# llrtt/G-NeRF

Measured on NVIDIA B200. Metric: ray-samples/sec, higher is better.
Workload: dtype f32

## Files before the change

### g-nerf_b200/csrc/tpr_render_ws.cuh

```cuda
#pragma once
#include <cuda_runtime.h>
#include <stdint.h>
#include <stddef.h>
#include <string.h>
#include <cuda_bf16.h>
#include "triplane_b200.h"
#include "tpr_render.cuh"
#include "tpr_ws.cuh"

namespace tpr {
using namespace tc;

namespace ws {

struct Barriers {
  uint64_t a1_full[kBufs];
  uint64_t a1_free[kBufs];
  uint64_t d1_full;
  uint64_t a2_full;
  uint64_t coarse_ready[kCtx];
  uint64_t fine_ready[kCtx];
  uint64_t csig_ready[kCtx];
  uint64_t fsig_ready[kCtx];
  uint64_t stg_full[2];
};

struct Ctx { float* dep; float* sig; float* u; float* ray; int* rk; };

struct Geom { long long ray0; int n, rstride, nr; };
__device__ __forceinline__ Geom group_geom(const RenderArgs& a, unsigned grp, int R) {
  Geom g;
  const unsigned tpi = (unsigned)a.tiles_per_img;
  const unsigned n = grp / tpi, gi = grp - n * tpi;
  const bool colm = a.col_w > 0;
  const unsigned cw = colm ? (unsigned)a.col_w : 1u;
  const unsigned gy = gi / cw, gx = gi - gy * cw;
  g.n = (int)n;
  g.ray0 = (long long)n * a.rays_per_img + (colm ? (long long)(gy * R * cw + gx) : (long long)gi * R);
  g.rstride = (int)cw;
  g.nr = colm ? R : (int)min((long long)R, a.rays_per_img - (long long)gi * R);
  return g;
}

template <int MODE, bool TRAIN = false>
__device__ __forceinline__ void gather_tile(const RenderArgs& a, float* a1_hi, const float* __restrict__ img,
                                            const Ctx& cx, Tap2* tw, int nr, int Dx, int off, int S, int t, int dpt_shift,
                                            int warp, int lane, long long ray0 = 0, int rstride = 0) {
#ifndef TPR_GATHER_256
  const int grp = lane >> 3, sub = lane & 7;
#endif
  const int dpt = 1 << dpt_shift;
  {
    const int s = lane / 3, p = lane - s * 3;
    const int row = warp * 8 + s;
    const int r = row >> dpt_shift, di = t * dpt + (row & (dpt - 1));
    if (lane < 24 && r < nr && di < Dx) {
      const float d = cx.dep[r * S + off + di];
      const float* ry = cx.ray + r * 8;
      const float px = __fmul_rn(__fadd_rn(ry[0], __fmul_rn(d, ry[3])), a.box_scale);
      const float py = __fmul_rn(__fadd_rn(ry[1], __fmul_rn(d, ry[4])), a.box_scale);
      const float pz = __fmul_rn(__fadd_rn(ry[2], __fmul_rn(d, ry[5])), a.box_scale);
      Taps tp;
      plane_taps(p == 2 ? pz : px, p == 0 ? py : (p == 1 ? pz : px), a.H, a.W, tp);
      const int po = p * a.H * a.W * kC;
      *reinterpret_cast<uint4*>(tw[lane].off) = make_uint4((unsigned)(tp.off[0] + po) >> 2, (unsigned)(tp.off[1] + po) >> 2,
                                                           (unsigned)(tp.off[2] + po) >> 2, (unsigned)(tp.off[3] + po) >> 2);
      *reinterpret_cast<float4*>(tw[lane].w2) = make_float4(tp.w[0], tp.w[0], tp.w[1], tp.w[1]);
      *reinterpret_cast<float4*>(tw[lane].w2 + 4) = make_float4(tp.w[2], tp.w[2], tp.w[3], tp.w[3]);
    }
  }
  __syncwarp();
#ifdef TPR_GATHER_256
  {
    const int s = lane >> 2, sub4 = lane & 3;
    const ulonglong2* base = reinterpret_cast<const ulonglong2*>(img) + 2 * sub4;
    asm volatile("" : "+l"(base));
    const int row = warp * 8 + s;
    const int r = row >> dpt_shift, di = t * dpt + (row & (dpt - 1));
    if (r < nr && di < Dx) {
      float4* keep = (TRAIN && a.sample_features != nullptr)
          ? reinterpret_cast<float4*>(a.sample_features + ((ray0 + (long long)r * rstride) * S + off + di) * 32) + 2 * sub4 : nullptr;
      blend_sample8<MODE>(a1_hi, base, tw + s * 3, row, sub4, keep);
    }
  }
#else
  const ulonglong2* base = reinterpret_cast<const ulonglong2*>(img) + sub;
  asm volatile("" : "+l"(base));
#pragma unroll 1
  for (int rd = 0; rd < 2; ++rd) {
#if !defined(TPR_ROWS_INTERLEAVED) || TPR_ROWS_INTERLEAVED
    const int s = (grp & 1) | ((grp >> 1) << 2) | (rd << 1);
#else
    const int s = rd * 4 + grp;
#endif
    const int row = warp * 8 + s;
    const int r = row >> dpt_shift, di = t * dpt + (row & (dpt - 1));
    if (r < nr && di < Dx) {
      const Tap2* te = tw + s * 3;
      float4* keep = (TRAIN && a.sample_features != nullptr)
          ? reinterpret_cast<float4*>(a.sample_features + ((ray0 + (long long)r * rstride) * S + off + di) * 32) + sub : nullptr;
      blend_sample<MODE>(a1_hi, base, te, row, sub, keep);
    }
  }
#endif
  __syncwarp();
}

template <int MODE, int E, int ER, bool PROF, bool TRAIN = false>
__global__ void __launch_bounds__(kThreads, 1) render_ws_kernel(const RenderArgs a) {
  extern __shared__ uint8_t smem_raw[];
  uint8_t* base = smem_raw + ((1024u - (smem_u32(smem_raw) & 1023u)) & 1023u);
  Tiles<MODE>& tl = *reinterpret_cast<Tiles<MODE>*>(base);
  Tap2* taps = reinterpret_cast<Tap2*>(base + sizeof(Tiles<MODE>));
  float* fl = reinterpret_cast<float*>(base + sizeof(Tiles<MODE>) + sizeof(Tap2) * kGatherWarps * 24);
  const int R = a.R, Dc = a.Dc, Df = a.Df, S = Dc + Df;
  const int dpt_shift = R == 8 ? 4 : 5, dpt = 1 << dpt_shift;
  const int ctx_floats = 2 * R * S + R * Df + R * 8 + (R == 4 ? R * Df : 0);
  float* scratch = fl + kCtx * ctx_floats;
  auto ctx_of = [&](int gi) {
    float* p = fl + (gi & (kCtx - 1)) * ctx_floats;
    Ctx c; c.dep = p; c.sig = p + R * S; c.u = c.sig + R * S; c.ray = c.u + R * Df; c.rk = reinterpret_cast<int*>(c.ray + R * 8);
    return c;
  };
  __shared__ Barriers bars;
  __shared__ uint32_t tmem_base_sm;
  __shared__ unsigned range_sm[2];
  __shared__ unsigned freed_warps;
  __shared__ int slot_tab[kCtx][16];
  __shared__ long long prof[24];
  const bool profiling = PROF && a.dbg != nullptr && blockIdx.x == 0;
#define PROF_T0() long long pt0_ = (PROF && profiling) ? clock64() : 0
#define PROF_ADD(i, cond) do { if (PROF && profiling && (cond)) { const long long now_ = clock64(); prof[i] += now_ - pt0_; pt0_ = now_; } } while (0)
  const int tid = threadIdx.x, warp = __shfl_sync(0xffffffffu, tid >> 5, 0), lane = tid & 31;
  const bool sleep_waits = (a.variant & 2) != 0;
#define WAIT_SLACK(bar, par) do { if (sleep_waits) mbar_wait_sleep(bar, par); else mbar_wait_parked(bar, par); } while (0)

  const int nf_host = a.Df;
  if (tid == 0) {
    range_sm[0] = 0xffffffffu; range_sm[1] = 0u;
    for (int b = 0; b < kBufs; ++b) { mbar_init(&bars.a1_full[b], kGatherWarps); mbar_init(&bars.a1_free[b], 1); }
    mbar_init(&bars.d1_full, 1); mbar_init(&bars.a2_full, kDecodeWarps);
    mbar_init(&bars.stg_full[0], 1); mbar_init(&bars.stg_full[1], 1);
    for (int c = 0; c < kCtx; ++c) {
      mbar_init(&bars.coarse_ready[c], kRayWarps); mbar_init(&bars.fine_ready[c], kRayWarps);
      mbar_init(&bars.csig_ready[c], nf_host == 0 ? 5 : 4); mbar_init(&bars.fsig_ready[c], 5);
    }
    freed_warps = 0u;
    for (int i = 0; i < 24; ++i) prof[i] = 0;
    fence_mbar_init();
  }
  if (warp == 0) { tmem_alloc(&tmem_base_sm, 512); tmem_relinquish(); }
  for (int i = tid; i < (int)(sizeof(tl.a1) / 16); i += kThreads) reinterpret_cast<float4*>(tl.a1)[i] = make_float4(0.f, 0.f, 0.f, 0.f);
  stage_weights<MODE>(a.dec, tl);
  fence_proxy_async_smem();
  tcgen05_fence_before();
  __syncthreads();
  tcgen05_fence_after();
  const uint32_t tmem = __shfl_sync(0xffffffffu, tmem_base_sm, 0);
  const uint32_t lane_base = (uint32_t)((warp & 3) * 32) << 16;

  const int nc = (Dc + dpt - 1) >> dpt_shift, nf = Df > 0 ? (Df + dpt - 1) >> dpt_shift : 0;
  const int G = (int)((a.n_tiles - blockIdx.x + gridDim.x - 1) / gridDim.x);
  const size_t img_stride = (size_t)3 * a.H * a.W * kC;
  const bool per_ray = a.rs != nullptr;

  if (warp < kGatherWarps) {
    Tap2* tw = taps + warp * 24;
    int b = 0; uint32_t ph = 0;
    for (int step = 0; step <= G; ++step) {
#pragma unroll 1
      for (int jb = 0; jb < 2; ++jb) {
        const int pass = jb;
        int gi;
        if (pass == 0) { if (step >= G) continue; gi = step; }
        else { if (step < 1 || nf == 0) continue; gi = step - 1; }
        const Geom gg = group_geom(a, blockIdx.x + (unsigned)gi * gridDim.x, R);
        const Ctx cx = ctx_of(gi);
        const uint32_t cpar = (uint32_t)(gi >> 2) & 1u;
        PROF_T0();
        WAIT_SLACK(pass == 0 ? &bars.coarse_ready[gi & 3] : &bars.fine_ready[gi & 3], cpar);
        PROF_ADD(pass, tid == 0);
        const float* img = a.planes + (size_t)((unsigned)gg.n % (unsigned)a.plane_sets) * img_stride;
        const int T = pass == 0 ? nc : nf, Dx = pass == 0 ? Dc : Df, off = pass == 0 ? 0 : Dc;
#pragma unroll 1
        for (int t = 0; t < T; ++t) {
          WAIT_SLACK(&bars.a1_free[b], ph ^ 1u);
          PROF_ADD(2, tid == 0);
          gather_tile<MODE, TRAIN>(a, tl.a1[b][0], img, cx, tw, gg.nr, Dx, off, S, t, dpt_shift, warp, lane, gg.ray0, gg.rstride);
          fence_proxy_async_smem();
          __syncwarp();
          if (lane == 0) mbar_arrive(&bars.a1_full[b]);
          PROF_ADD(3, tid == 0);
          if (++b == kBufs) { b = 0; ph ^= 1u; }
        }
      }
    }
  } else if (warp < kFirstRayWarp) {
    const int dw = warp - kFirstDecodeWarp, q = dw & 3, h = dw >> 2;
    const bool issuer = dw == 0;
    uint32_t pt = 0;
    const uint32_t dbase = smem_desc_lo(smem_u32(&tl));
    uint32_t free_mask = (1u << Cols<MODE>::ns) - 1u;
    int freed_groups = 0;
    int b = 0; uint32_t ph = 0;
    for (int step = 0; step <= G; ++step) {
#pragma unroll 1
      for (int jb = 0; jb < 2; ++jb) {
        const int pass = jb;
        int gi;
        if (pass == 0) { if (step >= G) continue; gi = step; }
        else { if (step < 1 || nf == 0) continue; gi = step - 1; }
        const Geom gg = group_geom(a, blockIdx.x + (unsigned)gi * gridDim.x, R);
        const Ctx cx = ctx_of(gi);
        const int T = pass == 0 ? nc : nf, Dx = pass == 0 ? Dc : Df, off = pass == 0 ? 0 : Dc;
#pragma unroll 1
        for (int t = 0; t < T; ++t) {
          PROF_T0();
          const bool pl = dw == 0 && lane == 0;
          const uint32_t st = tmem;
          if (issuer) {
            mbar_wait_parked(&bars.a1_full[b], ph);
            PROF_ADD(4, pl);
            tcgen05_fence_after();
            const int bu = __shfl_sync(0xffffffffu, b, 0);
            if (elect_one_sync()) {
              issue_layer1<MODE>(dbase, bu, st);
              mma_commit(&bars.a1_free[b]);
              mma_commit(&bars.d1_full);
            }
            __syncwarp();
          }
          if (++b == kBufs) { b = 0; ph ^= 1u; }
          int slot = 0;
          if (issuer) {
            do {
              const int fg = (int)(*reinterpret_cast<volatile unsigned*>(&freed_warps) / kRayWarps);
              for (; freed_groups < fg; ++freed_groups)
                for (int i = 0; i < nc + nf; ++i) free_mask |= 1u << slot_tab[freed_groups & (kCtx - 1)][i];
            } while (free_mask == 0u);
            __threadfence_block();
            slot = __shfl_sync(0xffffffffu, __ffs(free_mask) - 1, 0);
            free_mask &= ~(1u << slot);
            if (lane == 0) slot_tab[gi & (kCtx - 1)][(pass == 0 ? 0 : nc) + t] = slot;
          }
          PROF_ADD(5, pl);
          mbar_wait_parked(&bars.d1_full, pt);
          PROF_ADD(6, pl);
          tcgen05_fence_after();
          const float sgp = epilogue1<MODE>(tl, st, lane_base, h);
          tcgen05_fence_before();
          __syncwarp();
          if (lane == 0) mbar_arrive(&bars.a2_full);
          PROF_ADD(7, pl);
          if (issuer) {
            mbar_wait_parked(&bars.a2_full, pt);
            PROF_ADD(8, pl);
            tcgen05_fence_after();
            if (elect_one_sync()) {
              issue_layer2<MODE>(dbase, st, tmem + Cols<MODE>::slots + slot * kSlotCols);
              if (t == T - 1 && (pass == 1 || nf == 0)) mma_commit(pass == 0 ? &bars.csig_ready[gi & 3] : &bars.fsig_ready[gi & 3]);
            }
            __syncwarp();
          }
          PROF_ADD(9, pl);
          float* ps = tl.psig + (pt ? kRows : 0);
          if (h == 1) ps[q * 32 + lane] = sgp;
          named_bar_sync(3 + q, 64);
          if (h == 0) {
            const int row = q * 32 + lane, r = row >> dpt_shift, di = t * dpt + (row & (dpt - 1));
            if (r < gg.nr && di < Dx) cx.sig[r * S + off + di] = sgp + ps[row] + tl.bias2[kNc];
          }
          PROF_ADD(10, pl);
          if (h == 0 && t == T - 1) {
            __syncwarp();
            if (lane == 0) mbar_arrive(pass == 0 ? &bars.csig_ready[gi & 3] : &bars.fsig_ready[gi & 3]);
          }
          pt ^= 1u;
          PROF_ADD(11, pl);
        }
      }
    }
  } else {
    const int rw = warp - kFirstRayWarp, rtid = tid - kFirstRayWarp * 32;
    const int q = rw & 3, hc = rw >> 2;
    constexpr int kRayThreads = kRayWarps * 32;
    float* wa = scratch; float* wb = wa + R * S; float* wc = wb + R * S; float* rayw = wc + R * S;
    float mn = __int_as_float(0x7f800000), mx = -__int_as_float(0x7f800000);
    float smn = mn, smx = mx;
    int cur_slot = 0;
#define RAY_SYNC() named_bar_sync(2, kRayThreads)

    const bool pl = rtid == 0;
    const bool bulk = a.bulk_inputs != 0;
    float* stg_jit = rayw + R; float* stg_u = stg_jit + 2 * R * Dc; float* stg_ray = stg_u + 2 * R * Df;
    int* hist = reinterpret_cast<int*>(stg_ray + R * 8 + 8);
    const bool merge = R == 4 && nf > 0 && (Df & 3) == 0 && a.variant != 3;
    const bool split = merge && a.noise_c == nullptr && (a.variant & 16) == 0;
    float* so_a = split ? reinterpret_cast<float*>(hist + R * (Dc + 4)) : wa;
    float* so_b = split ? so_a + R * S : wb;
    auto prefetch = [&](int gi) {
      const Geom gg = group_geom(a, blockIdx.x + (unsigned)gi * gridDim.x, R);
      if (rtid < gg.nr * 6) {
        const int r = rtid / 6, c = rtid - r * 6;
        const long long g = gg.ray0 + (long long)r * gg.rstride;
        cp_async4(stg_ray + rtid, c < 3 ? a.origins + g * 3 + c : a.dirs + g * 3 + c - 3);
      }
      float* sj = stg_jit + (gi & 1) * R * Dc; float* su = stg_u + (gi & 1) * R * Df;
      if (bulk) {
        if (rtid == 0) {
          mbar_arrive_expect_tx(&bars.stg_full[gi & 1], (uint32_t)(gg.nr * (Dc + Df)) * 4u);
          for (int r = 0; r < gg.nr; ++r) {
            const long long g = gg.ray0 + (long long)r * gg.rstride;
            bulk_copy_g2s(sj + r * Dc, a.jitter + g * Dc, (uint32_t)Dc * 4u, &bars.stg_full[gi & 1]);
            if (Df > 0) bulk_copy_g2s(su + r * Df, a.u + g * Df, (uint32_t)Df * 4u, &bars.stg_full[gi & 1]);
          }
        }
      } else {
        for (int s = rtid; s < gg.nr * Dc; s += kRayThreads) {
          const int r = s / Dc, k = s - r * Dc;
          cp_async4(sj + s, a.jitter + (gg.ray0 + (long long)r * gg.rstride) * Dc + k);
        }
        for (int s = rtid; s < gg.nr * Df; s += kRayThreads) {
          const int r = s / Df, k = s - r * Df;
          cp_async4(su + s, a.u + (gg.ray0 + (long long)r * gg.rstride) * Df + k);
        }
      }
      cp_async_commit();
    };
    auto setup = [&](int gi) {
      PROF_T0();
      const Geom gg = group_geom(a, blockIdx.x + (unsigned)gi * gridDim.x, R);
      const Ctx cx = ctx_of(gi);
      cp_async_wait_all();
      if (bulk) mbar_wait_parked(&bars.stg_full[gi & 1], (uint32_t)(gi >> 1) & 1u);
      const float* sj = stg_jit + (gi & 1) * R * Dc; const float* su = stg_u + (gi & 1) * R * Df;
      if (rtid < gg.nr * 6) { const int r = rtid / 6; cx.ray[r * 8 + (rtid - r * 6)] = stg_ray[rtid]; }
      for (int s = rtid; s < gg.nr * Dc; s += kRayThreads) {
        const int r = s / Dc, k = s - r * Dc;
        const long long g = gg.ray0 + (long long)r * gg.rstride;
        const float lo = per_ray ? __ldg(a.rs + g) : a.ray_start, hi = per_ray ? __ldg(a.re + g) : a.ray_end;
        cx.dep[r * S + k] = coarse_depth(a, k, sj[s], lo, hi, per_ray);
      }
      for (int s = rtid; s < gg.nr * Df; s += kRayThreads) cx.u[s] = su[s];
      __syncwarp();
      if (lane == 0) mbar_arrive(&bars.coarse_ready[gi & 3]);
      PROF_ADD(12, pl);
    };

    auto resample = [&](int gi) {
      const Geom gg = group_geom(a, blockIdx.x + (unsigned)gi * gridDim.x, R);
      const Ctx cx = ctx_of(gi);
      PROF_T0();
      WAIT_SLACK(&bars.csig_ready[gi & 3], (uint32_t)(gi >> 2) & 1u);
      PROF_ADD(13, pl);
      if (a.noise_c != nullptr) {
        add_density_noise(a, a.noise_c, cx.sig, S, 0, Dc, gg.nr * Dc, gg.ray0, gg.rstride, rtid, kRayThreads);
        RAY_SYNC();
      }
      for (int r = rw; r < gg.nr; r += kRayWarps)
        warp_resample_ray(a, cx.dep + r * S, cx.sig + r * S, wa + r * S, wb + r * S, wc + r * S, cx.dep + r * S + Dc,
                          gg.ray0 + (long long)r * gg.rstride, lane, cx.u + r * Df);
      if (!split && merge && rw >= 4 && rw - 4 < gg.nr) warp_rank_draws(cx.u + (rw - 4) * Df, cx.rk + (rw - 4) * Df, Df, lane);
      __syncwarp();
      if (lane == 0) mbar_arrive(&bars.fine_ready[gi & 3]);
      if (split && (a.variant & 32) == 0 && rw < gg.nr) warp_rank_draws(cx.u + rw * Df, cx.rk + rw * Df, Df, lane);
      PROF_ADD(14, pl);
    };

    auto sort_split = [&](int gi) {
      const Geom gg = group_geom(a, blockIdx.x + (unsigned)gi * gridDim.x, R);
      const Ctx cx = ctx_of(gi);
      PROF_T0();
      mbar_wait_parked(&bars.fsig_ready[gi & 3], (uint32_t)(gi >> 2) & 1u);
      PROF_ADD(15, pl);
      if (range_slot(a, gg.n) != cur_slot) { range_fold(a, cur_slot, smn, smx, mn, mx, lane); cur_slot = range_slot(a, gg.n); }
      const int r = rw - 4;
      if (r < gg.nr) {
        float wsum, dnum;
        bool pre = false;
        if (cx.rk[r * Df] >= 0)
          pre = warp_merge_scatter(cx.dep + r * S, cx.sig + r * S, cx.rk + r * Df, so_a + r * S, so_b + r * 2 * S, hist + r * (Dc + 4),
                                   S, Dc, lane);
        warp_sort_and_weights<E, true, ER>(cx.dep + r * S, cx.sig + r * S, so_a + r * S, nullptr, S, lane, wsum, dnum, smn, smx,
                                           so_b + r * 2 * S, pre);
        if (lane == 0) {
          const long long g = gg.ray0 + (long long)r * gg.rstride;
          rayw[r] = wsum;
          const float dq = dnum / wsum;
          a.depth[g] = dq;
          a.wsum[g] = wsum;
          for (int p = 0; p < a.peers.n; ++p) { a.peers.depth[p][g] = dq; a.peers.wsum[p][g] = wsum; }
        }
      }
      PROF_ADD(18, pl);
    };

    auto sort_composite = [&](int gi, bool sorted, const float* om_rows) {
      const Geom gg = group_geom(a, blockIdx.x + (unsigned)gi * gridDim.x, R);
      const Ctx cx = ctx_of(gi);
      PROF_T0();
      WAIT_SLACK(nf > 0 ? &bars.fsig_ready[gi & 3] : &bars.csig_ready[gi & 3], (uint32_t)(gi >> 2) & 1u);
      PROF_ADD(15, pl);
      if (a.noise_c != nullptr) {
        if (nf > 0) add_density_noise(a, a.noise_f, cx.sig, S, Dc, Df, gg.nr * Df, gg.ray0, gg.rstride, rtid, kRayThreads);
        else add_density_noise(a, a.noise_c, cx.sig, S, 0, Dc, gg.nr * Dc, gg.ray0, gg.rstride, rtid, kRayThreads);
        RAY_SYNC();
      }
      if (range_slot(a, gg.n) != cur_slot) { range_fold(a, cur_slot, smn, smx, mn, mx, lane); cur_slot = range_slot(a, gg.n); }
      const bool pairs = R == 4 && nf > 0 && (Dc & 31) == 0 && (Df & 7) == 0;
      for (int r = (pairs || merge) ? (rw & 3) : rw; !sorted && r < gg.nr; r += kRayWarps) {
        float wsum, dnum;
        bool pre = false;
        const bool mg = merge && cx.rk[r * Df] >= 0;
        if (mg) {
          if (rw >= 4) break;
          pre = warp_merge_scatter(cx.dep + r * S, cx.sig + r * S, cx.rk + r * Df, wa + r * S, wb + r * 2 * S, hist + r * (Dc + 4),
                                   S, Dc, lane);
          PROF_ADD(18, pl);
        } else if (!pairs && merge && rw >= 4) {
          break;
        } else if (pairs) {
          pre = pair_rank_scatter<ER>(cx.dep + r * S, cx.sig + r * S, wa + r * S, wb + r * 2 * S, S, Dc, lane, rw >> 2, 7 + r);
          if (rw >= 4) break;
          PROF_ADD(18, pl);
        }
        warp_sort_and_weights<E, true, ER>(cx.dep + r * S, cx.sig + r * S, wa + r * S, nullptr, S, lane, wsum, dnum, smn, smx,
                                       wb + r * 2 * S, pre);
        if (TRAIN && a.sample_sigma != nullptr) {
          float* dst = a.sample_sigma + (gg.ray0 + (long long)r * gg.rstride) * S;
          for (int p = lane; p < S; p += 32) dst[p] = cx.sig[r * S + p];
        }
        if (lane == 0) {
          const long long g = gg.ray0 + (long long)r * gg.rstride;
          rayw[r] = wsum;
          const float dq = dnum / wsum;
          a.depth[g] = dq;
          a.wsum[g] = wsum;
          for (int p = 0; p < a.peers.n; ++p) { a.peers.depth[p][g] = dq; a.peers.wsum[p][g] = wsum; }
        }
      }
      RAY_SYNC();
      PROF_ADD(16, pl);
      tcgen05_fence_after();
      const int row = q * 32 + lane, r = row >> dpt_shift, i = row & (dpt - 1);
      uint64_t acc2[8];
#pragma unroll
      for (int c = 0; c < 8; ++c) acc2[c] = 0ull;
      const uint64_t kOne2 = pack2(1.0f, 1.0f), kScale2 = pack2(1.002f, 1.002f), kShift2 = pack2(-0.001f, -0.001f);
#pragma unroll 1
      for (int sl = 0; sl < nc + nf; ++sl) {
        const bool fine = sl >= nc;
        const int tl_i = fine ? sl - nc : sl;
        const int slot = slot_tab[gi & (kCtx - 1)][sl];
        const int di = tl_i * dpt + i;
        const bool valid = r < gg.nr && di < (fine ? Df : Dc);
        const float om = valid ? om_rows[r * S + (fine ? Dc : 0) + di] : 0.0f;
        uint32_t v[16];
        tmem_ld16(tmem + Cols<MODE>::slots + slot * kSlotCols + lane_base + 16 * hc, v);
        tmem_wait_ld();
        const uint64_t om2 = pack2(om, om);
        ulonglong2* cdst = (TRAIN && a.sample_colours != nullptr && valid)
            ? reinterpret_cast<ulonglong2*>(a.sample_colours + ((gg.ray0 + (long long)r * gg.rstride) * 8 + 4 * hc) * (long long)S * 4) +
                  ((fine ? Dc : 0) + di)
            : nullptr;
        const int cstep = S;
#pragma unroll
        for (int c4 = 0; c4 < 4; ++c4) {
          const ulonglong2 bz = *reinterpret_cast<const ulonglong2*>(tl.bias2 + 16 * hc + 4 * c4);
          ulonglong2 cpair;
#pragma unroll
          for (int h2 = 0; h2 < 2; ++h2) {
            const int c = 4 * c4 + 2 * h2;
            float z0, z1;
            unpack2(add2(pack2(__uint_as_float(v[c]), __uint_as_float(v[c + 1])), h2 == 0 ? bz.x : bz.y), z0, z1);
            const uint64_t den = add2(pack2(ex2_fast(z0), ex2_fast(z1)), kOne2);
            float d0, d1;
            unpack2(den, d0, d1);
            const uint64_t col = fma2(pack2(rcp_fast(d0), rcp_fast(d1)), kScale2, kShift2);
            acc2[c >> 1] = fma2(om2, col, acc2[c >> 1]);
            if (h2 == 0) cpair.x = col; else cpair.y = col;
          }
          if (TRAIN && cdst != nullptr) cdst[c4 * cstep] = cpair;
        }
      }
      float acc[16];
#pragma unroll
      for (int c = 0; c < 8; ++c) unpack2(acc2[c], acc[2 * c], acc[2 * c + 1]);
      tcgen05_fence_before();
      __syncwarp();
      if (lane == 0) { __threadfence_block(); atomicAdd(&freed_warps, 1u); }
#pragma unroll
      for (int o = 1; o < 32; o <<= 1) {
        if (o < dpt) {
#pragma unroll
          for (int c = 0; c < 16; ++c) acc[c] += __shfl_xor_sync(kFull, acc[c], o);
        }
      }
      if (i == 0 && r < gg.nr) {
        const float wsr = rayw[r];
        long long cstride;
        float* dst1 = rgb_ptr(a, gg.ray0 + (long long)r * gg.rstride, gg.n, cstride);
        dst1 += 16 * hc * cstride;
#pragma unroll
        for (int c = 0; c < 16; ++c) {
          float v = acc[c];
          if (a.white_back) v = v + 1.0f - wsr;
          acc[c] = v * 2.0f - 1.0f;
        }
        const long long eoff = dst1 - a.rgb;
#pragma unroll 1
        for (int p = -1; p < a.peers.n; ++p) {
          float* d1 = p < 0 ? dst1 : a.peers.rgb[p] + eoff;
          if (a.nchw) {
#pragma unroll
            for (int c = 0; c < 16; ++c) d1[c * cstride] = acc[c];
          } else {
            float4* dst = reinterpret_cast<float4*>(d1);
#pragma unroll
            for (int c4 = 0; c4 < 4; ++c4) dst[c4] = make_float4(acc[4 * c4], acc[4 * c4 + 1], acc[4 * c4 + 2], acc[4 * c4 + 3]);
          }
        }
      }
      RAY_SYNC();
      PROF_ADD(17, pl);
    };

    prefetch(0); setup(0);
    if (G > 1) { prefetch(1); setup(1); }
    if (G > 2) prefetch(2);
    for (int g = 0; g < G; ++g) {
      if (split) {
        if (rw < 4) resample(g);
        else {
          if (lane == 0) mbar_arrive(&bars.fine_ready[g & 3]);
          if (g >= 1) sort_split(g - 1);
          if ((a.variant & 32) != 0) {
            const Geom gg = group_geom(a, blockIdx.x + (unsigned)g * gridDim.x, R);
            const Ctx cx = ctx_of(g);
            if (rw - 4 < gg.nr) warp_rank_draws(cx.u + (rw - 4) * Df, cx.rk + (rw - 4) * Df, Df, lane);
          }
        }
        RAY_SYNC();
      } else if (nf > 0) {
        resample(g);
      }
      if (g + 2 < G) { setup(g + 2); if (g + 3 < G) prefetch(g + 3); }
      if (nf > 0) { if (g >= 1) sort_composite(g - 1, split, so_a); }
      else sort_composite(g, false, wa);
    }
    if (nf > 0) {
      if (split) { if (rw >= 4) sort_split(G - 1); RAY_SYNC(); }
      sort_composite(G - 1, split, so_a);
    }
    range_fold(a, cur_slot, smn, smx, mn, mx, lane);
    mn = warp_min(mn); mx = warp_max(mx);
    if (lane == 0 && mn <= mx) {
      atomicMin(&range_sm[0], float_to_ordered(mn));
      atomicMax(&range_sm[1], float_to_ordered(mx));
    }
  }
  tcgen05_fence_before();
  __syncthreads();
  if (tid == 0 && range_sm[0] <= range_sm[1]) {
    atomicMin(a.range_enc + 0, range_sm[0]);
    atomicMax(a.range_enc + 1, range_sm[1]);
  }
  if (warp == 0) { tcgen05_fence_after(); tmem_dealloc(tmem, 512); }
  if (PROF && profiling && tid < 24) a.dbg[tid] = prof[tid];
}

template <int MODE>
static size_t smem_bytes(int R, int S, int Df) {
  return 1024 + sizeof(Tiles<MODE>) + sizeof(Tap2) * kGatherWarps * 24 +
         sizeof(float) * ((size_t)kCtx * (2 * R * S + R * Df + R * 8 + (R == 4 ? R * Df : 0)) + (size_t)3 * R * S + R +
                          (size_t)2 * R * S + R * 8 + 8 + (R == 4 ? R * (S - Df + 4) + (size_t)3 * R * S : 0));
}

typedef void (*Kernel)(const RenderArgs);
template <int MODE> Kernel kernel_small(int S, bool prof, bool train);
template <int MODE> Kernel kernel_large(int S, bool prof);

}
}
```

### g-nerf_b200/csrc/tpr_ws.cuh

```cuda
#pragma once
#include <cuda_runtime.h>
#include <stdint.h>
#include <stddef.h>
#include <cuda_bf16.h>
#include <cuda_fp16.h>
#include "tpr_device.cuh"
#include "tpr_tc.cuh"

namespace tpr {
namespace ws {
using namespace tc;

constexpr int kGatherWarps = 16, kDecodeWarps = 8, kRayWarps = 8;
constexpr int kThreads = 32 * (kGatherWarps + kDecodeWarps + kRayWarps);
constexpr int kFirstDecodeWarp = kGatherWarps, kFirstRayWarp = kGatherWarps + kDecodeWarps;
constexpr int kRows = 128;
constexpr int kN1 = 64, kNc = 32;
#ifndef TPR_A1_BUFS
#define TPR_A1_BUFS 3
#endif
constexpr int kBufs = TPR_A1_BUFS;
constexpr int kCtx = 4;
constexpr int kSlotCols = 32;

constexpr uint32_t kStageCols = 64;
template <int MODE> struct Cols;
template <> struct Cols<1> { static constexpr uint32_t a2hi = 64, a2lo = 64, a2step = 8, slots = 96; static constexpr int ns = 13; };
template <> struct Cols<2> { static constexpr uint32_t a2hi = 0, a2lo = 8, a2step = 16, slots = 64; static constexpr int ns = 14; };

template <int MODE> struct Tiles;
template <> struct Tiles<1> {
  float a1[kBufs][1][kRows * 32];
  float b1[1][kN1 * 32];
  float b2c[1][1][kNc * 32];
  float bias1[kN1];
  float w2s[kN1];
  float bias2[kNc + 4];
  float psig[2 * kRows];
};
template <> struct Tiles<2> {
  float a1[kBufs][1][kRows * 32];
  float b1[1][kN1 * 32];
  float b2c[2][1][kNc * 32];
  float bias1[kN1];
  float w2s[kN1];
  float bias2[kNc + 4];
  float psig[2 * kRows];
};

__device__ __forceinline__ void st_swz_f32(float* tile, int row, int k, float v) {
  tile[row * 32 + ((((k >> 2) ^ (row & 7)) << 2) | (k & 3))] = v;
}
__device__ __forceinline__ void st_swz_bf16(float* tile, int row, int k, float v) {
  reinterpret_cast<__nv_bfloat16*>(tile)[row * 64 + ((((k >> 3) ^ (row & 7)) << 3) | (k & 7))] = __float2bfloat16_rn(v);
}

__device__ __forceinline__ void st_swz_f16(float* tile, int row, int k, __half v) {
  reinterpret_cast<__half*>(tile)[row * 64 + ((((k >> 3) ^ (row & 7)) << 3) | (k & 7))] = v;
}
__device__ __forceinline__ void split_f16(float x, __half& hi, __half& lo) {
  hi = __float2half_rn(fminf(fmaxf(x, -65504.0f), 65504.0f));
  lo = __float2half_rn(x - __half2float(hi));
}
__device__ __forceinline__ uint32_t pack_f16x2(float lo_elem, float hi_elem) {
  uint32_t r;
  asm("cvt.rn.satfinite.f16x2.f32 %0, %1, %2;" : "=r"(r) : "f"(hi_elem), "f"(lo_elem));
  return r;
}
__device__ __forceinline__ void unpack_f16x2(uint32_t v, float& lo_elem, float& hi_elem) {
  const __half2 h = *reinterpret_cast<const __half2*>(&v);
  const float2 f = __half22float2(h);
  lo_elem = f.x; hi_elem = f.y;
}

template <int MODE>
__device__ void stage_weights(const float* __restrict__ dec, Tiles<MODE>& tl) {
  const int tid = threadIdx.x, nthreads = blockDim.x;
  for (int i = tid; i < kN1 * 32; i += nthreads) {
    const int n = i >> 5, k = i & 31;
    const float w = dec[kW1tOff + k * kHid + n] * kLog2e;
    if (MODE == 1) st_swz_bf16(tl.b1[0], n, k, w);
    else { __half hi, lo; split_f16(w, hi, lo); st_swz_f16(tl.b1[0], n, k, hi); st_swz_f16(tl.b1[0], n, 32 + k, lo); }
  }
  for (int i = tid; i < kNc * 64; i += nthreads) {
    const int n = i >> 6, k = i & 63;
    const float w = -dec[kW2tOff + k * kOutPad + n + 1];
    if (MODE == 1) st_swz_bf16(tl.b2c[0][0], n, k, w);
    else { __half hi, lo; split_f16(w, hi, lo); st_swz_f16(tl.b2c[0][0], n, k, hi); st_swz_f16(tl.b2c[MODE == 2 ? 1 : 0][0], n, k, lo); }
  }
  for (int i = tid; i < kN1; i += nthreads) {
    tl.bias1[i] = dec[kB1Off + i] * kLog2e;
    tl.w2s[i] = dec[kW2tOff + i * kOutPad] * kLn2;
  }
  for (int i = tid; i < kNc + 1; i += nthreads) tl.bias2[i] = i < kNc ? -kLog2e * dec[kB2Off + 1 + i] : dec[kB2Off];
}

struct __align__(16) Tap2 { uint32_t off[4]; float w2[8]; };

template <int MODE>
__device__ __forceinline__ void blend_sample(float* a1_hi, const ulonglong2* base, const Tap2* te, int row, int sub,
                                             float4* keep = nullptr) {
  uint64_t f01 = 0ull, f23 = 0ull;
#pragma unroll 1
  for (int p = 0; p < 3; ++p) {
    const uint4 o = *reinterpret_cast<const uint4*>(te[p].off);
    const ulonglong2 wa = *reinterpret_cast<const ulonglong2*>(te[p].w2), wb = *reinterpret_cast<const ulonglong2*>(te[p].w2 + 4);
#ifdef TPR_SKIP_PADDING_PLANES
    if ((wa.x | wa.y | wb.x | wb.y) == 0ull) continue;
#endif
    const ulonglong2 v0 = __ldg(base + o.x), v1 = __ldg(base + o.y), v2 = __ldg(base + o.z), v3 = __ldg(base + o.w);
    uint64_t a01 = fma2(wa.x, v0.x, 0ull), a23 = fma2(wa.x, v0.y, 0ull);
    a01 = fma2(wa.y, v1.x, a01); a23 = fma2(wa.y, v1.y, a23);
    a01 = fma2(wb.x, v2.x, a01); a23 = fma2(wb.x, v2.y, a23);
    a01 = fma2(wb.y, v3.x, a01); a23 = fma2(wb.y, v3.y, a23);
    f01 = add2(f01, a01); f23 = add2(f23, a23);
  }
  float4 f;
  unpack2(f01, f.x, f.y); unpack2(f23, f.z, f.w);
  if (keep != nullptr) *keep = f;
  if (MODE == 1) {
    uint2 pk = make_uint2(pack_bf16(f.x, f.y), pack_bf16(f.z, f.w));
    uint8_t* dst = reinterpret_cast<uint8_t*>(a1_hi) + row * 128 + ((((sub >> 1) ^ (row & 7)) << 4) | ((sub & 1) << 3));
    *reinterpret_cast<uint2*>(dst) = pk;
  } else {
    const uint2 hi = make_uint2(pack_f16x2(f.x, f.y), pack_f16x2(f.z, f.w));
    float h0, h1, h2, h3;
    unpack_f16x2(hi.x, h0, h1); unpack_f16x2(hi.y, h2, h3);
    const uint2 lo = make_uint2(pack_f16x2(f.x - h0, f.y - h1), pack_f16x2(f.z - h2, f.w - h3));
    uint8_t* rowp = reinterpret_cast<uint8_t*>(a1_hi) + row * 128 + ((sub & 1) << 3);
    *reinterpret_cast<uint2*>(rowp + (((sub >> 1) ^ (row & 7)) << 4)) = hi;
    *reinterpret_cast<uint2*>(rowp + ((((sub >> 1) + 4) ^ (row & 7)) << 4)) = lo;
  }
}

struct U256 { uint64_t a, b, c, d; };
__device__ __forceinline__ U256 ldg256(const ulonglong2* p) {
  U256 r;
  asm volatile("ld.global.nc.v4.b64 {%0,%1,%2,%3}, [%4];" : "=l"(r.a), "=l"(r.b), "=l"(r.c), "=l"(r.d) : "l"(p));
  return r;
}
template <int MODE>
__device__ __forceinline__ void blend_sample8(float* a1_hi, const ulonglong2* base, const Tap2* te, int row, int sub,
                                              float4* keep = nullptr) {
  uint64_t f0 = 0ull, f1 = 0ull, f2 = 0ull, f3 = 0ull;
#pragma unroll 1
  for (int p = 0; p < 3; ++p) {
    const uint4 o = *reinterpret_cast<const uint4*>(te[p].off);
    const ulonglong2 wa = *reinterpret_cast<const ulonglong2*>(te[p].w2), wb = *reinterpret_cast<const ulonglong2*>(te[p].w2 + 4);
    const U256 v0 = ldg256(base + o.x), v1 = ldg256(base + o.y), v2 = ldg256(base + o.z), v3 = ldg256(base + o.w);
    uint64_t a0 = fma2(wa.x, v0.a, 0ull), a1 = fma2(wa.x, v0.b, 0ull), a2 = fma2(wa.x, v0.c, 0ull), a3 = fma2(wa.x, v0.d, 0ull);
    a0 = fma2(wa.y, v1.a, a0); a1 = fma2(wa.y, v1.b, a1); a2 = fma2(wa.y, v1.c, a2); a3 = fma2(wa.y, v1.d, a3);
    a0 = fma2(wb.x, v2.a, a0); a1 = fma2(wb.x, v2.b, a1); a2 = fma2(wb.x, v2.c, a2); a3 = fma2(wb.x, v2.d, a3);
    a0 = fma2(wb.y, v3.a, a0); a1 = fma2(wb.y, v3.b, a1); a2 = fma2(wb.y, v3.c, a2); a3 = fma2(wb.y, v3.d, a3);
    f0 = add2(f0, a0); f1 = add2(f1, a1); f2 = add2(f2, a2); f3 = add2(f3, a3);
  }
  float4 fa, fb;
  unpack2(f0, fa.x, fa.y); unpack2(f1, fa.z, fa.w); unpack2(f2, fb.x, fb.y); unpack2(f3, fb.z, fb.w);
  if (keep != nullptr) { keep[0] = fa; keep[1] = fb; }
  if (MODE == 1) {
    uint4 pk = make_uint4(pack_bf16(fa.x, fa.y), pack_bf16(fa.z, fa.w), pack_bf16(fb.x, fb.y), pack_bf16(fb.z, fb.w));
    uint8_t* dst = reinterpret_cast<uint8_t*>(a1_hi) + row * 128 + ((sub ^ (row & 7)) << 4);
    *reinterpret_cast<uint4*>(dst) = pk;
  } else {
    const uint4 hi = make_uint4(pack_f16x2(fa.x, fa.y), pack_f16x2(fa.z, fa.w), pack_f16x2(fb.x, fb.y), pack_f16x2(fb.z, fb.w));
    float h[8];
    unpack_f16x2(hi.x, h[0], h[1]); unpack_f16x2(hi.y, h[2], h[3]); unpack_f16x2(hi.z, h[4], h[5]); unpack_f16x2(hi.w, h[6], h[7]);
    const uint4 lo = make_uint4(pack_f16x2(fa.x - h[0], fa.y - h[1]), pack_f16x2(fa.z - h[2], fa.w - h[3]),
                                pack_f16x2(fb.x - h[4], fb.y - h[5]), pack_f16x2(fb.z - h[6], fb.w - h[7]));
    uint8_t* rowp = reinterpret_cast<uint8_t*>(a1_hi) + row * 128;
    *reinterpret_cast<uint4*>(rowp + ((sub ^ (row & 7)) << 4)) = hi;
    *reinterpret_cast<uint4*>(rowp + (((sub + 4) ^ (row & 7)) << 4)) = lo;
  }
}

#define TPR_OFF16(member) ((uint32_t)(offsetof(Tiles<MODE>, member) >> 4))
#define TPR_D(lo) desc_sw128_from_lo(lo)
template <int MODE>
__device__ __forceinline__ void issue_layer1(uint32_t dlo, int buf, uint32_t d1) {
  constexpr uint32_t kTile16 = (kRows * 32 * 4) >> 4;
  const uint32_t ah = dlo + TPR_OFF16(a1) + (uint32_t)buf * kTile16;
  const uint32_t bh = dlo + TPR_OFF16(b1);
  if (MODE == 1) {
    const uint32_t idesc = instr_desc(kFmtBF16, 128, kN1);
#pragma unroll
    for (int ks = 0; ks < 2; ++ks) mma_f16_ss(d1, TPR_D(ah + 2 * ks), TPR_D(bh + 2 * ks), idesc, ks > 0);
  } else {
    const uint32_t idesc = instr_desc(kFmtF16, 128, kN1);
#pragma unroll
    for (int ks = 0; ks < 2; ++ks) {
      mma_f16_ss(d1, TPR_D(ah + 2 * ks), TPR_D(bh + 2 * ks), idesc, ks > 0);
      mma_f16_ss(d1, TPR_D(ah + 4 + 2 * ks), TPR_D(bh + 2 * ks), idesc, true);
      mma_f16_ss(d1, TPR_D(ah + 2 * ks), TPR_D(bh + 4 + 2 * ks), idesc, true);
    }
  }
}

template <int MODE>
__device__ __forceinline__ void issue_layer2(uint32_t dlo, uint32_t st, uint32_t dc) {
  const uint32_t bh = dlo + TPR_OFF16(b2c);
  constexpr uint32_t kB16 = (kNc * 32 * 4) >> 4;
  if (MODE == 1) {
    const uint32_t ic = instr_desc(kFmtBF16, 128, kNc);
#pragma unroll
    for (int ks = 0; ks < 4; ++ks) mma_f16_ts(dc, st + Cols<MODE>::a2hi + ks * Cols<MODE>::a2step, TPR_D(bh + 2 * ks), ic, ks > 0);
  } else {
    const uint32_t ic = instr_desc(kFmtF16, 128, kNc);
#pragma unroll
    for (int ks = 0; ks < 4; ++ks) {
      mma_f16_ts(dc, st + Cols<MODE>::a2hi + ks * 16, TPR_D(bh + 2 * ks), ic, ks > 0);
      mma_f16_ts(dc, st + Cols<MODE>::a2lo + ks * 16, TPR_D(bh + 2 * ks), ic, true);
      mma_f16_ts(dc, st + Cols<MODE>::a2hi + ks * 16, TPR_D(bh + kB16 + 2 * ks), ic, true);
    }
  }
}

template <int MODE, bool kStoreA2 = true>
__device__ __forceinline__ float epilogue1(const Tiles<MODE>& tl, uint32_t st, uint32_t lane_base, int h) {
  uint64_t sg2 = 0ull;
  const uint64_t kOne2 = pack2(1.0f, 1.0f);
#pragma unroll
  for (int c = 0; c < 2; ++c) {
    const int col = 32 * h + 16 * c;
    uint32_t r[16];
    tmem_ld16(st + lane_base + col, r);
    tmem_wait_ld();
#pragma unroll
    for (int half = 0; half < 2; ++half) {
      uint64_t act2[4];
#pragma unroll
      for (int i4 = 0; i4 < 2; ++i4) {
        const int o = 8 * half + 4 * i4;
        const ulonglong2 b = *reinterpret_cast<const ulonglong2*>(tl.bias1 + col + o);
        const ulonglong2 w = *reinterpret_cast<const ulonglong2*>(tl.w2s + col + o);
#pragma unroll
        for (int h2 = 0; h2 < 2; ++h2) {
          const uint64_t xs2 = add2(pack2(__uint_as_float(r[o + 2 * h2]), __uint_as_float(r[o + 2 * h2 + 1])), h2 == 0 ? b.x : b.y);
          float x0, x1, y0, y1;
          unpack2(xs2, x0, x1);
          unpack2(add2(pack2(ex2_fast(x0), ex2_fast(x1)), kOne2), y0, y1);
          y0 = x0 > 20.0f * kLog2e ? x0 : lg2_fast(y0);
          y1 = x1 > 20.0f * kLog2e ? x1 : lg2_fast(y1);
          act2[2 * i4 + h2] = pack2(y0, y1);
          sg2 = fma2(act2[2 * i4 + h2], h2 == 0 ? w.x : w.y, sg2);
        }
      }
      if (!kStoreA2) {
      } else if (MODE == 1) {
        uint32_t pk[4];
#pragma unroll
        for (int i = 0; i < 4; ++i) { float y0, y1; unpack2(act2[i], y0, y1); pk[i] = pack_bf16(y0, y1); }
        tmem_st4(st + Cols<MODE>::a2hi + lane_base + ((col + 8 * half) >> 1), pk);
      } else {
        uint32_t hi[4], lo[4];
#pragma unroll
        for (int i = 0; i < 4; ++i) {
          float y0, y1, h0, h1;
          unpack2(act2[i], y0, y1);
          hi[i] = pack_f16x2(y0, y1);
          unpack_f16x2(hi[i], h0, h1);
          lo[i] = pack_f16x2(y0 - h0, y1 - h1);
        }
        tmem_st4(st + Cols<MODE>::a2hi + lane_base + col + 4 * half, hi);
        tmem_st4(st + Cols<MODE>::a2lo + lane_base + col + 4 * half, lo);
      }
    }
  }
  if (kStoreA2) tmem_wait_st();
  float s0, s1;
  unpack2(sg2, s0, s1);
  return s0 + s1;
}

}
}
```

### profiles/phase_timing.py

```python
import os, sys, importlib
os.environ['TPR_PHASE_TIMING'] = '1'
sys.path.insert(0, os.path.dirname(os.path.dirname(os.path.abspath(__file__))))
import torch, numpy as np
pkg = importlib.import_module('g-nerf_b200')
import bench
dev = torch.device('cuda:0')
planes_h, c2w, K = bench.make_inputs(torch, 100)
dec = bench.make_decoder(torch, pkg, dev, 0)
R, S = pkg.ImportanceRenderer(), pkg.RaySampler()
planes = planes_h.to(dev); o, d = S(c2w.to(dev), K.to(dev), 128)
WS = ['GATHER wait coarse_ready', 'GATHER wait fine_ready', 'GATHER wait a1_free', 'GATHER gather+publish',
      'DECODE wait a1_full (issuer)', 'DECODE issue M1 + slot', 'DECODE wait d1_full', 'DECODE epilogue1', 'DECODE wait a2_full (issuer)',
      'DECODE issue M2', 'DECODE sigma halves exchange (named barrier)', 'DECODE publish sigma (arrive)', 'RAYS setup', 'RAYS wait csig', 'RAYS resample',
      'RAYS wait fsig', 'RAYS sort+march', 'RAYS composite', 'RAYS   (merge / pair rank count at 96+96: part of the sort, not counted in sort+march)']
D = int(os.environ.get('TPR_PT_DEPTH', '48'))
RPG = 8 if D <= 48 else 4
for mode in sys.argv[1:] or ['fp32']:
    opts = dict(bench.OPTS, decoder_precision=mode, depth_resolution=D, depth_resolution_importance=D)
    for _ in range(3): R(planes, dec, o, d, opts)
    torch.cuda.synchronize()
    t = R.last_scratch[64:64 + 24 * 8].view(torch.int64).cpu().numpy()
    ngroups = 16384 * 8 / RPG / 148
    names = WS
    print(mode, 'CTA0 cycles per group (', int(ngroups), 'groups )')
    for n, v in zip(names, t): print(f'  {n:32s} {int(v / ngroups):7d}')
```

Before: 5.234 billion.

## Merge gather and decode warps into three round-robin teams owning A1 buffers

Replaces the separate 16 gather warps and 8 decode warps with three 8-warp teams. Each team gathers a tile into its own A1 buffer, issues the layer-1 and layer-2 MMAs, and runs the epilogue. Tiles are assigned to teams round-robin, and a stage_free barrier chain serialises MMA issue across teams. This removes the producer/consumer handoff and the fixed split of warps between roles, so every warp can both gather and decode. In exchange, each team now carries the full per-tile latency itself, the tensor-core issue order is serialised, and the sigma and slot barrier counts become more intricate.

New measurement: 5.032 billion, median of 6. -3.9%, worse.

```diff
diff --git a/g-nerf_b200/csrc/tpr_render_ws.cuh b/g-nerf_b200/csrc/tpr_render_ws.cuh
--- a/g-nerf_b200/csrc/tpr_render_ws.cuh
+++ b/g-nerf_b200/csrc/tpr_render_ws.cuh
@@ -13,11 +13,13 @@
 
 namespace ws {
 
+constexpr int kTeams = 3, kTeamWarps = 8, kTeamBar = 11;
+static_assert(kTeams * kTeamWarps == kFirstRayWarp, "warps below the ray warps form the teams");
+static_assert(kBufs == kTeams, "team k owns A1 buffer k");
+
 struct Barriers {
-  uint64_t a1_full[kBufs];
-  uint64_t a1_free[kBufs];
-  uint64_t d1_full;
-  uint64_t a2_full;
+  uint64_t d1_full[kTeams];
+  uint64_t stage_free[kTeams];
   uint64_t coarse_ready[kCtx];
   uint64_t fine_ready[kCtx];
   uint64_t csig_ready[kCtx];
@@ -112,7 +114,8 @@
   uint8_t* base = smem_raw + ((1024u - (smem_u32(smem_raw) & 1023u)) & 1023u);
   Tiles<MODE>& tl = *reinterpret_cast<Tiles<MODE>*>(base);
   Tap2* taps = reinterpret_cast<Tap2*>(base + sizeof(Tiles<MODE>));
-  float* fl = reinterpret_cast<float*>(base + sizeof(Tiles<MODE>) + sizeof(Tap2) * kGatherWarps * 24);
+  float* team_psig = reinterpret_cast<float*>(taps + kFirstRayWarp * 24);
+  float* fl = team_psig + kTeams * kRows;
   const int R = a.R, Dc = a.Dc, Df = a.Df, S = Dc + Df;
   const int dpt_shift = R == 8 ? 4 : 5, dpt = 1 << dpt_shift;
   const int ctx_floats = 2 * R * S + R * Df + R * 8 + (R == 4 ? R * Df : 0);
@@ -125,7 +128,8 @@
   __shared__ Barriers bars;
   __shared__ uint32_t tmem_base_sm;
   __shared__ unsigned range_sm[2];
-  __shared__ unsigned freed_warps;
+  __shared__ unsigned freed_warps, free_mask_sm;
+  __shared__ int freed_groups_sm;
   __shared__ int slot_tab[kCtx][16];
   __shared__ long long prof[24];
   const bool profiling = PROF && a.dbg != nullptr && blockIdx.x == 0;
@@ -135,19 +139,19 @@
   const bool sleep_waits = (a.variant & 2) != 0;
 #define WAIT_SLACK(bar, par) do { if (sleep_waits) mbar_wait_sleep(bar, par); else mbar_wait_parked(bar, par); } while (0)
 
-  const int nf_host = a.Df;
+  const int nc = (Dc + dpt - 1) >> dpt_shift, nf = Df > 0 ? (Df + dpt - 1) >> dpt_shift : 0;
   if (tid == 0) {
     range_sm[0] = 0xffffffffu; range_sm[1] = 0u;
-    for (int b = 0; b < kBufs; ++b) { mbar_init(&bars.a1_full[b], kGatherWarps); mbar_init(&bars.a1_free[b], 1); }
-    mbar_init(&bars.d1_full, 1); mbar_init(&bars.a2_full, kDecodeWarps);
+    for (int k = 0; k < kTeams; ++k) { mbar_init(&bars.d1_full[k], 1); mbar_init(&bars.stage_free[k], 1); }
     mbar_init(&bars.stg_full[0], 1); mbar_init(&bars.stg_full[1], 1);
     for (int c = 0; c < kCtx; ++c) {
       mbar_init(&bars.coarse_ready[c], kRayWarps); mbar_init(&bars.fine_ready[c], kRayWarps);
-      mbar_init(&bars.csig_ready[c], nf_host == 0 ? 5 : 4); mbar_init(&bars.fsig_ready[c], 5);
-    }
-    freed_warps = 0u;
+      mbar_init(&bars.csig_ready[c], nf == 0 ? 5 * nc : 4 * nc); mbar_init(&bars.fsig_ready[c], 4 * nf + nc + nf);
+    }
+    freed_warps = 0u; free_mask_sm = (1u << Cols<MODE>::ns) - 1u; freed_groups_sm = 0;
     for (int i = 0; i < 24; ++i) prof[i] = 0;
     fence_mbar_init();
+    mbar_arrive(&bars.stage_free[0]);
   }
   if (warp == 0) { tmem_alloc(&tmem_base_sm, 512); tmem_relinquish(); }
   for (int i = tid; i < (int)(sizeof(tl.a1) / 16); i += kThreads) reinterpret_cast<float4*>(tl.a1)[i] = make_float4(0.f, 0.f, 0.f, 0.f);
@@ -159,14 +163,19 @@
   const uint32_t tmem = __shfl_sync(0xffffffffu, tmem_base_sm, 0);
   const uint32_t lane_base = (uint32_t)((warp & 3) * 32) << 16;
 
-  const int nc = (Dc + dpt - 1) >> dpt_shift, nf = Df > 0 ? (Df + dpt - 1) >> dpt_shift : 0;
   const int G = (int)((a.n_tiles - blockIdx.x + gridDim.x - 1) / gridDim.x);
   const size_t img_stride = (size_t)3 * a.H * a.W * kC;
   const bool per_ray = a.rs != nullptr;
 
-  if (warp < kGatherWarps) {
+  if (warp < kFirstRayWarp) {
+    const int team = warp / kTeamWarps, wt = warp - team * kTeamWarps, q = wt & 3, h = wt >> 2;
+    const bool issuer = wt == 0, pl = tid == 0;
     Tap2* tw = taps + warp * 24;
-    int b = 0; uint32_t ph = 0;
+    float* ps = team_psig + team * kRows;
+    const uint32_t dbase = smem_desc_lo(smem_u32(&tl));
+    const uint32_t st = tmem;
+    int jm = 0;
+    uint32_t ph = 0;
     for (int step = 0; step <= G; ++step) {
 #pragma unroll 1
       for (int jb = 0; jb < 2; ++jb) {
@@ -174,108 +183,82 @@
         int gi;
         if (pass == 0) { if (step >= G) continue; gi = step; }
         else { if (step < 1 || nf == 0) continue; gi = step - 1; }
+        const int T = pass == 0 ? nc : nf, Dx = pass == 0 ? Dc : Df, off = pass == 0 ? 0 : Dc;
+        const int t0 = team >= jm ? team - jm : team - jm + kTeams;
+        jm = (jm + T) % kTeams;
+        if (t0 >= T) continue;
         const Geom gg = group_geom(a, blockIdx.x + (unsigned)gi * gridDim.x, R);
         const Ctx cx = ctx_of(gi);
-        const uint32_t cpar = (uint32_t)(gi >> 2) & 1u;
         PROF_T0();
-        WAIT_SLACK(pass == 0 ? &bars.coarse_ready[gi & 3] : &bars.fine_ready[gi & 3], cpar);
-        PROF_ADD(pass, tid == 0);
+        WAIT_SLACK(pass == 0 ? &bars.coarse_ready[gi & 3] : &bars.fine_ready[gi & 3], (uint32_t)(gi >> 2) & 1u);
+        PROF_ADD(pass, pl);
         const float* img = a.planes + (size_t)((unsigned)gg.n % (unsigned)a.plane_sets) * img_stride;
-        const int T = pass == 0 ? nc : nf, Dx = pass == 0 ? Dc : Df, off = pass == 0 ? 0 : Dc;
+        uint64_t* sig_bar = pass == 0 ? &bars.csig_ready[gi & 3] : &bars.fsig_ready[gi & 3];
+        uint64_t* slots_bar = nf == 0 ? &bars.csig_ready[gi & 3] : &bars.fsig_ready[gi & 3];
 #pragma unroll 1
-        for (int t = 0; t < T; ++t) {
-          WAIT_SLACK(&bars.a1_free[b], ph ^ 1u);
-          PROF_ADD(2, tid == 0);
-          gather_tile<MODE, TRAIN>(a, tl.a1[b][0], img, cx, tw, gg.nr, Dx, off, S, t, dpt_shift, warp, lane, gg.ray0, gg.rstride);
+        for (int t = t0; t < T; t += kTeams) {
+#pragma unroll 1
+          for (int p8 = 0; p8 < 2; ++p8)
+            gather_tile<MODE, TRAIN>(a, tl.a1[team][0], img, cx, tw, gg.nr, Dx, off, S, t, dpt_shift, 2 * wt + p8, lane, gg.ray0,
+                                     gg.rstride);
           fence_proxy_async_smem();
-          __syncwarp();
-          if (lane == 0) mbar_arrive(&bars.a1_full[b]);
-          PROF_ADD(3, tid == 0);
-          if (++b == kBufs) { b = 0; ph ^= 1u; }
-        }
-      }
-    }
-  } else if (warp < kFirstRayWarp) {
-    const int dw = warp - kFirstDecodeWarp, q = dw & 3, h = dw >> 2;
-    const bool issuer = dw == 0;
-    uint32_t pt = 0;
-    const uint32_t dbase = smem_desc_lo(smem_u32(&tl));
-    uint32_t free_mask = (1u << Cols<MODE>::ns) - 1u;
-    int freed_groups = 0;
-    int b = 0; uint32_t ph = 0;
-    for (int step = 0; step <= G; ++step) {
-#pragma unroll 1
-      for (int jb = 0; jb < 2; ++jb) {
-        const int pass = jb;
-        int gi;
-        if (pass == 0) { if (step >= G) continue; gi = step; }
-        else { if (step < 1 || nf == 0) continue; gi = step - 1; }
-        const Geom gg = group_geom(a, blockIdx.x + (unsigned)gi * gridDim.x, R);
-        const Ctx cx = ctx_of(gi);
-        const int T = pass == 0 ? nc : nf, Dx = pass == 0 ? Dc : Df, off = pass == 0 ? 0 : Dc;
-#pragma unroll 1
-        for (int t = 0; t < T; ++t) {
-          PROF_T0();
-          const bool pl = dw == 0 && lane == 0;
-          const uint32_t st = tmem;
+          PROF_ADD(2, pl);
+          named_bar_sync(kTeamBar + team, kTeamWarps * 32);
+          PROF_ADD(3, pl);
+          int slot = 0;
           if (issuer) {
-            mbar_wait_parked(&bars.a1_full[b], ph);
+            mbar_wait_parked(&bars.stage_free[team], ph);
             PROF_ADD(4, pl);
             tcgen05_fence_after();
-            const int bu = __shfl_sync(0xffffffffu, b, 0);
             if (elect_one_sync()) {
-              issue_layer1<MODE>(dbase, bu, st);
-              mma_commit(&bars.a1_free[b]);
-              mma_commit(&bars.d1_full);
+              issue_layer1<MODE>(dbase, team, st);
+              mma_commit(&bars.d1_full[team]);
             }
             __syncwarp();
-          }
-          if (++b == kBufs) { b = 0; ph ^= 1u; }
-          int slot = 0;
-          if (issuer) {
+            PROF_ADD(5, pl);
+            unsigned fm = *reinterpret_cast<volatile unsigned*>(&free_mask_sm);
+            int fgd = *reinterpret_cast<volatile int*>(&freed_groups_sm);
             do {
               const int fg = (int)(*reinterpret_cast<volatile unsigned*>(&freed_warps) / kRayWarps);
-              for (; freed_groups < fg; ++freed_groups)
-                for (int i = 0; i < nc + nf; ++i) free_mask |= 1u << slot_tab[freed_groups & (kCtx - 1)][i];
-            } while (free_mask == 0u);
+              for (; fgd < fg; ++fgd)
+                for (int i = 0; i < nc + nf; ++i) fm |= 1u << slot_tab[fgd & (kCtx - 1)][i];
+            } while (fm == 0u);
             __threadfence_block();
-            slot = __shfl_sync(0xffffffffu, __ffs(free_mask) - 1, 0);
-            free_mask &= ~(1u << slot);
-            if (lane == 0) slot_tab[gi & (kCtx - 1)][(pass == 0 ? 0 : nc) + t] = slot;
-          }
-          PROF_ADD(5, pl);
-          mbar_wait_parked(&bars.d1_full, pt);
+            slot = __shfl_sync(0xffffffffu, __ffs(fm) - 1, 0);
+            if (lane == 0) {
+              slot_tab[gi & (kCtx - 1)][(pass == 0 ? 0 : nc) + t] = slot;
+              free_mask_sm = fm & ~(1u << slot); freed_groups_sm = fgd;
+            }
+            __syncwarp();
+            __threadfence_block();
+            PROF_ADD(9, pl);
+          }
+          mbar_wait_parked(&bars.d1_full[team], ph);
           PROF_ADD(6, pl);
           tcgen05_fence_after();
           const float sgp = epilogue1<MODE>(tl, st, lane_base, h);
           tcgen05_fence_before();
-          __syncwarp();
-          if (lane == 0) mbar_arrive(&bars.a2_full);
+          if (h == 1) ps[q * 32 + lane] = sgp;
           PROF_ADD(7, pl);
+          named_bar_sync(kTeamBar + team, kTeamWarps * 32);
+          PROF_ADD(8, pl);
           if (issuer) {
-            mbar_wait_parked(&bars.a2_full, pt);
-            PROF_ADD(8, pl);
             tcgen05_fence_after();
             if (elect_one_sync()) {
               issue_layer2<MODE>(dbase, st, tmem + Cols<MODE>::slots + slot * kSlotCols);
-              if (t == T - 1 && (pass == 1 || nf == 0)) mma_commit(pass == 0 ? &bars.csig_ready[gi & 3] : &bars.fsig_ready[gi & 3]);
+              mma_commit(&bars.stage_free[team == kTeams - 1 ? 0 : team + 1]);
+              mma_commit(slots_bar);
             }
             __syncwarp();
-          }
-          PROF_ADD(9, pl);
-          float* ps = tl.psig + (pt ? kRows : 0);
-          if (h == 1) ps[q * 32 + lane] = sgp;
-          named_bar_sync(3 + q, 64);
+            PROF_ADD(10, pl);
+          }
           if (h == 0) {
             const int row = q * 32 + lane, r = row >> dpt_shift, di = t * dpt + (row & (dpt - 1));
             if (r < gg.nr && di < Dx) cx.sig[r * S + off + di] = sgp + ps[row] + tl.bias2[kNc];
-          }
-          PROF_ADD(10, pl);
-          if (h == 0 && t == T - 1) {
             __syncwarp();
-            if (lane == 0) mbar_arrive(pass == 0 ? &bars.csig_ready[gi & 3] : &bars.fsig_ready[gi & 3]);
-          }
-          pt ^= 1u;
+            if (lane == 0) mbar_arrive(sig_bar);
+          }
+          ph ^= 1u;
           PROF_ADD(11, pl);
         }
       }
@@ -571,7 +554,7 @@
 
 template <int MODE>
 static size_t smem_bytes(int R, int S, int Df) {
-  return 1024 + sizeof(Tiles<MODE>) + sizeof(Tap2) * kGatherWarps * 24 +
+  return 1024 + sizeof(Tiles<MODE>) + sizeof(Tap2) * kFirstRayWarp * 24 + sizeof(float) * kTeams * kRows +
          sizeof(float) * ((size_t)kCtx * (2 * R * S + R * Df + R * 8 + (R == 4 ? R * Df : 0)) + (size_t)3 * R * S + R +
                           (size_t)2 * R * S + R * 8 + 8 + (R == 4 ? R * (S - Df + 4) + (size_t)3 * R * S : 0));
 }
diff --git a/g-nerf_b200/csrc/tpr_ws.cuh b/g-nerf_b200/csrc/tpr_ws.cuh
--- a/g-nerf_b200/csrc/tpr_ws.cuh
+++ b/g-nerf_b200/csrc/tpr_ws.cuh
@@ -13,13 +13,10 @@
 
 constexpr int kGatherWarps = 16, kDecodeWarps = 8, kRayWarps = 8;
 constexpr int kThreads = 32 * (kGatherWarps + kDecodeWarps + kRayWarps);
-constexpr int kFirstDecodeWarp = kGatherWarps, kFirstRayWarp = kGatherWarps + kDecodeWarps;
+constexpr int kFirstRayWarp = kGatherWarps + kDecodeWarps;
 constexpr int kRows = 128;
 constexpr int kN1 = 64, kNc = 32;
-#ifndef TPR_A1_BUFS
-#define TPR_A1_BUFS 3
-#endif
-constexpr int kBufs = TPR_A1_BUFS;
+constexpr int kBufs = 3;
 constexpr int kCtx = 4;
 constexpr int kSlotCols = 32;
 
diff --git a/profiles/compare_dumps.py b/profiles/compare_dumps.py
--- /dev/null
+++ b/profiles/compare_dumps.py
@@ -0,0 +1,13 @@
+import os, sys
+import numpy as np
+a, b = sys.argv[1:3]
+bad = 0
+for f in sorted(os.listdir(a)):
+    if not f.endswith('.npy'):
+        continue
+    x, y = np.load(os.path.join(a, f)), np.load(os.path.join(b, f))
+    same = x.shape == y.shape and np.array_equal(x.view(np.uint32), y.view(np.uint32))
+    diff = float(np.nanmax(np.abs(x.astype(np.float64) - y))) if x.shape == y.shape else float('nan')
+    print(f'{a} vs {b}: {f:16s} {"bit-equal" if same else "DIFFERS"}  max-abs {diff:.3g}')
+    bad += not same
+sys.exit(1 if bad else 0)
diff --git a/profiles/outputs_dump.py b/profiles/outputs_dump.py
--- /dev/null
+++ b/profiles/outputs_dump.py
@@ -0,0 +1,22 @@
+import importlib, os, sys
+sys.path.insert(0, os.path.dirname(os.path.dirname(os.path.abspath(__file__))))
+import numpy as np
+import torch
+import bench
+pkg = importlib.import_module('g-nerf_b200')
+out = sys.argv[1]
+n, res, dc, df = (int(x) for x in sys.argv[2:6])
+mode = sys.argv[6] if len(sys.argv) > 6 else 'fp32'
+dev = torch.device('cuda:0')
+planes_h, c2w, K = bench.make_inputs(torch, 100, n_img=n)
+dec = bench.make_decoder(torch, pkg, dev, 0)
+R, S = pkg.ImportanceRenderer(), pkg.RaySampler()
+planes = planes_h.to(dev); o, d = S(c2w.to(dev), K.to(dev), res)
+opts = dict(bench.OPTS, decoder_precision=mode, depth_resolution=dc, depth_resolution_importance=df)
+torch.manual_seed(0)
+rgb, depth, wsum = R(pkg.pack_planes(planes), dec, o, d, opts)
+torch.cuda.synchronize()
+os.makedirs(out, exist_ok=True)
+for name, t in (('rgb', rgb), ('depth', depth), ('weight_sum', wsum)):
+    np.save(os.path.join(out, name + '.npy'), t.float().cpu().numpy())
+print(out, tuple(rgb.shape), 'finite:', bool(torch.isfinite(rgb).all()))
diff --git a/profiles/phase_timing.py b/profiles/phase_timing.py
--- a/profiles/phase_timing.py
+++ b/profiles/phase_timing.py
@@ -9,9 +9,10 @@
 dec = bench.make_decoder(torch, pkg, dev, 0)
 R, S = pkg.ImportanceRenderer(), pkg.RaySampler()
 planes = planes_h.to(dev); o, d = S(c2w.to(dev), K.to(dev), 128)
-WS = ['GATHER wait coarse_ready', 'GATHER wait fine_ready', 'GATHER wait a1_free', 'GATHER gather+publish',
-      'DECODE wait a1_full (issuer)', 'DECODE issue M1 + slot', 'DECODE wait d1_full', 'DECODE epilogue1', 'DECODE wait a2_full (issuer)',
-      'DECODE issue M2', 'DECODE sigma halves exchange (named barrier)', 'DECODE publish sigma (arrive)', 'RAYS setup', 'RAYS wait csig', 'RAYS resample',
+WS = ['TEAM wait coarse_ready', 'TEAM wait fine_ready', 'TEAM gather', 'TEAM barrier: tile gathered',
+      'TEAM wait stage free (issuer)', 'TEAM issue M1 (issuer)', 'TEAM wait d1_full', 'TEAM epilogue1',
+      'TEAM barrier: activations + sigma halves', 'TEAM colour slot (issuer)', 'TEAM issue M2 + commits (issuer)',
+      'TEAM publish sigma (arrive)', 'RAYS setup', 'RAYS wait csig', 'RAYS resample',
       'RAYS wait fsig', 'RAYS sort+march', 'RAYS composite', 'RAYS   (merge / pair rank count at 96+96: part of the sort, not counted in sort+march)']
 D = int(os.environ.get('TPR_PT_DEPTH', '48'))
 RPG = 8 if D <= 48 else 4
```
